# Enigmatisms/NeRF

Measured on AMD Instinct MI355X. Metric: rays/s (64+128 samples), 800x800, higher is better.
Workload: dtype bf16

## Files before the change

nerf_amd/csrc/mlp_core.h:

```cpp
#pragma once
#include "device_common.h"
#include "host_common.h"
#include "mlp_layout.h"

extern __shared__ __attribute__((aligned(16))) char smem[];

namespace {


struct PBF16 {
    using BReg = bf16x8;
    static constexpr int PREC = NERF_AMD_BF16;
    static constexpr int NW = MLP_NW_BF16;
    static constexpr int NT = 1;
    static constexpr int FRAG_BYTES = 1024;
    static constexpr int FPC = MLP_CHUNK_BYTES / FRAG_BYTES;
    using AReg = bf16x8;
    static constexpr int DEPTH = 4;
    static DEVINL AReg load_a(uint32_t frag_addr) { return *reinterpret_cast<const bf16x8*>(smem + frag_addr); }
    static DEVINL f32x16 mma(const AReg& a, const BReg& b, f32x16 acc) {
        return __builtin_amdgcn_mfma_f32_32x32x16_bf16(a, b, acc, 0, 0, 0);
    }
    template <int POS>
    static DEVINL f32x16 mma_pos(const AReg& a, const BReg& b, f32x16 acc) {
// ... 111 lines not shown
    const uint32_t m = __builtin_bit_cast(uint32_t, __builtin_elementwise_max(m01, m23));
    const uint32_t top = (m & 0xffffu) > (m >> 16) ? (m & 0xffffu) : (m >> 16);
    const uint32_t ex = top >> 7;
    return ex > 8u ? ex - 7u : 1u;
}
DEVINL u32x2 f8_encode_group(const bf16x8& v, uint32_t E) {
    const float scale = __builtin_bit_cast(float, E << 23);
    const u32x4 d = __builtin_bit_cast(u32x4, v);
    s16x2 lo = {0, 0}, hi = {0, 0};
    lo = __builtin_amdgcn_cvt_scalef32_pk_fp8_bf16(lo, __builtin_bit_cast(bf16x2, (uint32_t)d[0]), scale, false);
    lo = __builtin_amdgcn_cvt_scalef32_pk_fp8_bf16(lo, __builtin_bit_cast(bf16x2, (uint32_t)d[1]), scale, true);
    hi = __builtin_amdgcn_cvt_scalef32_pk_fp8_bf16(hi, __builtin_bit_cast(bf16x2, (uint32_t)d[2]), scale, false);
    hi = __builtin_amdgcn_cvt_scalef32_pk_fp8_bf16(hi, __builtin_bit_cast(bf16x2, (uint32_t)d[3]), scale, true);
    u32x2 r = {__builtin_bit_cast(uint32_t, lo), __builtin_bit_cast(uint32_t, hi)};
    return r;
}
DEVINL bf16x8 f8_decode_group(uint32_t lo, uint32_t hi, uint32_t E) {
    const float scale = __builtin_bit_cast(float, E << 23);
    const bf16x2 p0 = __builtin_amdgcn_cvt_scalef32_pk_bf16_fp8(lo, scale, false), p1 = __builtin_amdgcn_cvt_scalef32_pk_bf16_fp8(lo, scale, true);
    const bf16x2 p2 = __builtin_amdgcn_cvt_scalef32_pk_bf16_fp8(hi, scale, false), p3 = __builtin_amdgcn_cvt_scalef32_pk_bf16_fp8(hi, scale, true);
    bf16x8 r = {p0[0], p0[1], p1[0], p1[1], p2[0], p2[1], p3[0], p3[1]};
    return r;
}
DEVINL void f8_store_group(char* sub_base, int kg, int lane, const u32x2& v, uint32_t E, uint32_t scale_rec) {
    u32x2* dst = reinterpret_cast<u32x2*>(sub_base + (kg >> 1) * 1024 + lane * 16 + (kg & 1) * 8);
    __builtin_nontemporal_store(v, dst);
    *reinterpret_cast<unsigned char*>(smem + scale_rec + lane * 16 + kg) = (unsigned char)E;
}
DEVINL void f8_flush_scales(char* sub_base, int lane, uint32_t scale_rec) {
    const f32x4 v = *reinterpret_cast<const f32x4*>(smem + scale_rec + lane * 16);
    *reinterpret_cast<f32x4*>(sub_base + F8_SCALE_OFF + lane * 16) = v;
}

template <class P, int NSLOT = MLP_NSLOT>
struct WeightStream {
    static constexpr int LPW = (MLP_CHUNK_BYTES / 1024) / P::NW;
    const char* src;
    uint32_t n_chunks;
    uint32_t load_idx;
    uint32_t load_slot;
    uint32_t cur;
    uint32_t cur_slot;
    uint32_t wave_lds;
    typename P::AReg q[P::DEPTH];
    static DEVINL void dummy_sink(const bf16x8& d) { asm volatile("" ::"v"(d)); }
    template <class T> static DEVINL void dummy_sink(const T& d) { asm volatile("" ::"v"(d.lo), "v"(d.hi)); }
    DEVINL void issue() {
        const char* g = src + (size_t)load_idx * MLP_CHUNK_BYTES;
        const uint32_t dst = __builtin_amdgcn_readfirstlane(load_slot * MLP_CHUNK_BYTES + wave_lds);
#pragma unroll
        for (int i = 0; i < LPW; ++i) {
            unsigned keep;
            asm volatile("s_mov_b32 %0, m0\n\ts_mov_b32 m0, %2\n\ts_nop 0\n\tglobal_load_lds_dwordx4 %1, off\n\ts_mov_b32 m0, %0"
                         : "=&s"(keep)
                         : "v"(g + i * 1024), "s"(dst + i * 1024)
                         : "memory");
        }
        load_idx = (load_idx + 1 == n_chunks) ? 0u : load_idx + 1;
        load_slot = (load_slot + 1 == NSLOT) ? 0u : load_slot + 1;
    }
    static constexpr bool TWO_GROUPS = P::NW > 4;
    static constexpr int INFLIGHT = (TWO_GROUPS ? NSLOT - 5 : NSLOT - 4) * LPW;
    uint32_t late;

    DEVINL void init(const void* packed, uint32_t nchunks) {
        static_assert(NSLOT >= 6, "the protocol needs at least 6 ring slots");
        const int lane = lane_id();
        const int wave = __builtin_amdgcn_readfirstlane((int)(threadIdx.x >> 6));
        src = reinterpret_cast<const char*>(packed) + (size_t)wave * LPW * 1024 + lane * 16;
        wave_lds = wave * LPW * 1024;
        n_chunks = nchunks;
        load_idx = 0; load_slot = 0;
        cur_slot = 0;
        cur = lane * 16;
        late = __builtin_amdgcn_readfirstlane((P::NW > 4 && wave >= P::NW / 2) ? 1 : 0);
#pragma unroll
        for (int i = 0; i < NSLOT - 2; ++i) issue();
        asm volatile("s_waitcnt vmcnt(%0)" ::"n"(INFLIGHT) : "memory");
        __builtin_amdgcn_s_barrier();
        asm volatile("" ::: "memory");
#pragma unroll
        for (int i = 0; i < P::DEPTH; ++i) q[i] = P::load_a(cur + i * P::FRAG_BYTES);
        if (!late) {
            __builtin_amdgcn_s_barrier();
            asm volatile("" ::: "memory");
            issue();
        }
    }
    template <int F>
    DEVINL typename P::AReg next() {
        const typename P::AReg a = q[F % P::DEPTH];
        constexpr int G = F + P::DEPTH;
        if (G % P::FPC == 0) {
            cur_slot = (cur_slot + 1 == NSLOT) ? 0u : cur_slot + 1;
            cur = cur_slot * MLP_CHUNK_BYTES + lane_id() * 16;
            boundary<(G / P::FPC) & 1>();
        }
        q[F % P::DEPTH] = P::load_a(cur + (G % P::FPC) * P::FRAG_BYTES);
        return a;
    }
    template <int PARITY>
    DEVINL void boundary() {
        if constexpr (!TWO_GROUPS && PARITY != 0) {
            issue();
            return;
        }
        asm volatile("s_waitcnt vmcnt(%0)" ::"n"(INFLIGHT) : "memory");
        asm volatile("s_cmp_lg_u32 %0, %1\n\ts_cbranch_scc1 .Lnobar%=\n\ts_barrier\n.Lnobar%=:" ::"s"(__builtin_amdgcn_readfirstlane(late)), "n"(PARITY) : "memory", "scc");
        issue();
    }
    DEVINL void drain() {
        if (late) __builtin_amdgcn_s_barrier();
        asm volatile("s_waitcnt vmcnt(0)" ::: "memory");
    }
};

template <class P, int F0, int N, class WS, int I = 0>
DEVINL void skip_frags(WS& ws) {
    if constexpr (I < N) {
        const typename P::AReg a = ws.template next<F0 + I>();
        WS::dummy_sink(a);
        skip_frags<P, F0, N, WS, I + 1>(ws);
    }
}

// ... 135 lines not shown
```

nerf_amd/csrc/mlp_kernels.hip:

```cpp
#include "mlp_core.h"

namespace {

template <class P, int L, int NKG>
DEVINL void encode(float x, float y, float z, int h, typename P::BReg (&B)[NKG]) {
    if constexpr (P::FAST_PE) {
        float sv[3], cv[3];
        sincos_quadrant(x, sv[0], cv[0]); sincos_quadrant(y, sv[1], cv[1]); sincos_quadrant(z, sv[2], cv[2]);
#pragma unroll
        for (int f = 0; f < L; ++f) {
#pragma unroll
            for (int c = 0; c < 3; ++c) {
                const int q = 3 * f + c;
                P::set(B[q >> 3], q & 7, h ? cv[c] : sv[c]);
                if (f + 1 < L) {
                    const float s2 = 2.0f * sv[c];
                    const float ns = s2 * cv[c];
                    const float nc = __builtin_fmaf(-s2, sv[c], 1.0f);
                    sv[c] = ns; cv[c] = nc;
                }
            }
        }
#pragma unroll
        for (int q = 3 * L; q < 8 * NKG; ++q) {
// ... 143 lines not shown
    }
    float zv;
    if (s.z) zv = s.z[n * s.z_stride + si];
    else {
        const float uu = s.u ? s.u[n * s.S + si] : philox_u_strat(s.rng_seed, n + s.rng_ray_offset, si);
        zv = s.z_base[si] + uu * s.z_jitter;
    }
    r.x = ox + zv * r.dx; r.y = oy + zv * r.dy; r.z = oz + zv * r.dz;
    if (s.contract) contract_position(r);
    return r;
}

struct IpeSample { float mu[3], var[3], dx, dy, dz; };
DEVINL IpeSample fetch_sample_ipe(const nerf_amd_samples& s, int64_t m) {
    IpeSample r;
    int64_t n; int si;
    split_sample_index(s, m, n, si);
    const float* ry = s.rays + n * 6;
    const float* zz = s.z + n * s.z_stride + si;
    const float rr = s.ipe_radius;
    const ConeMoments c = cone_moments(zz[0], zz[1], (float)((double)rr * (double)rr));
    const float dn = s.ipe_dir_norm[0];
#pragma unroll
    for (int k = 0; k < 3; ++k) cone_mean_cov(c, ry[k], ry[3 + k], dn, r.mu[k], r.var[k]);
    r.dx = ry[3]; r.dy = ry[4]; r.dz = ry[5];
    if (s.contract) {
        Sample p{r.mu[0], r.mu[1], r.mu[2], 0.0f, 0.0f, 0.0f};
        contract_position(p);
        r.mu[0] = p.x; r.mu[1] = p.y; r.mu[2] = p.z;
    }
    return r;
}

constexpr uint32_t LDS_BIAS = MLP_RING_BYTES;
constexpr uint32_t LDS_STASH = MLP_RING_BYTES + 9216;
template <class P> constexpr uint32_t lds_dir() { return LDS_STASH + P::NW * P::NT * 4 * P::BREG_LDS; }
template <class P> constexpr uint32_t lds_tile() { return lds_dir<P>() + P::NW * P::NT * 1024; }
template <class P> constexpr uint32_t lds_total() { return lds_tile<P>() + P::NW * P::NT * 32 * 32 + P::NW * P::NT * 8 + 64; }

DEVINL void load_biases(const void* packed, size_t stream_bytes, int n_bias, uint32_t lds_off = MLP_RING_BYTES) {
    const float* b = reinterpret_cast<const float*>(reinterpret_cast<const char*>(packed) + stream_bytes);
    float* dst = reinterpret_cast<float*>(smem + lds_off);
    for (int i = threadIdx.x; i < n_bias; i += blockDim.x) dst[i] = b[i];
    __syncthreads();
}

struct ActDump {
    char* base;
    unsigned long long layer_stride;
    char* mask_base;
    unsigned long long mask_layer_stride;
};
template <class P>
DEVINL void dump_breg(const ActDump& d, int layer, int64_t subtile, int kg, int lane, const typename P::BReg& r) {
#ifndef ABL_NODUMPST
    P::store_global(d.base + (size_t)layer * d.layer_stride + ((size_t)subtile * 16 + kg) * (size_t)P::BREG_LDS, lane, r);
#endif
}

template <class P> constexpr uint32_t lds_maskacc() { return lds_total<P>(); }
template <class P> constexpr uint32_t lds_total_train() { return lds_total<P>() + P::NW * 2 * P::NT * 1024; }
template <class P> constexpr uint32_t lds_scaleacc() { return lds_total_train<P>(); }
template <class P> constexpr uint32_t lds_total_train_f8() { return lds_total_train<P>() + P::NW * 2 * P::NT * 1024; }
template <class P, bool F8>
DEVINL void dump_hidden(const ActDump& d, uint32_t sacc_wave, int layer, int64_t subtile, int t, int kg, int lane, const typename P::BReg& r) {
    if constexpr (F8) {
        const uint32_t E = f8_group_exponent<false>(r);
        f8_store_group(d.base + (size_t)layer * d.layer_stride + (size_t)subtile * F8_SUB_BYTES, kg, lane, f8_encode_group(r, E), E,
                       sacc_wave + ((layer & 1) * P::NT + t) * 1024);
    } else {
        dump_breg<P>(d, layer, subtile, kg, lane, r);
    }
}
DEVINL uint32_t breg_bits(const bf16x8& v) {
    typedef __attribute__((ext_vector_type(4))) uint32_t u32x4;
    const u32x4 d = __builtin_bit_cast(u32x4, v);
    uint32_t m = 0;
#pragma unroll
    for (int i = 0; i < 4; ++i) {
        const uint32_t x = d[i];
        uint32_t on;
        asm("v_pk_min_u16 %0, %1, %2" : "=v"(on) : "v"(x), "v"(0x00010001u));
        m |= on << i;
    }
    return m;
}
DEVINL uint32_t breg_bits(const f32x8& v) {
    uint32_t m = 0;
#pragma unroll
    for (int e = 0; e < 8; ++e) m |= (v[e] > 0.0f ? 1u : 0u) << ((e >> 1) + 16 * (e & 1));
    return m;
}
template <class P>
DEVINL void mask_or(uint32_t acc_wave, int layer, int t, int kg, int lane, const typename P::BReg& v) {
    unsigned* w = reinterpret_cast<unsigned*>(smem + acc_wave + ((layer & 1) * P::NT + t) * 1024 + lane * 16 + (kg >> 2) * 4);
    __hip_atomic_fetch_or(w, breg_bits(v) << (4 * (kg & 3)), __ATOMIC_RELAXED, __HIP_MEMORY_SCOPE_WORKGROUP);
}
template <class P, bool F8 = false>
DEVINL void mask_flush(const ActDump& d, uint32_t acc_wave, int layer, int64_t sub0, int lane, uint32_t sacc_wave = 0) {
    asm volatile("" ::: "memory");
#pragma unroll
    for (int t = 0; t < P::NT; ++t) {
        f32x4* rec = reinterpret_cast<f32x4*>(smem + acc_wave + ((layer & 1) * P::NT + t) * 1024 + lane * 16);
        const f32x4 v = *rec;
        *reinterpret_cast<f32x4*>(d.mask_base + (size_t)layer * d.mask_layer_stride + (size_t)(sub0 + t) * 1024 + lane * 16) = v;
        *rec = f32x4{0.0f, 0.0f, 0.0f, 0.0f};
        if constexpr (F8)
            f8_flush_scales(d.base + (size_t)layer * d.layer_stride + (size_t)(sub0 + t) * F8_SUB_BYTES, lane, sacc_wave + ((layer & 1) * P::NT + t) * 1024);
    }
    asm volatile("" ::: "memory");
}
template <class P>
DEVINL void mask_acc_init(uint32_t acc_wave, int lane) {
#pragma unroll
    for (int i = 0; i < 2 * P::NT; ++i) *reinterpret_cast<f32x4*>(smem + acc_wave + i * 1024 + lane * 16) = f32x4{0.0f, 0.0f, 0.0f, 0.0f};
}

template <class P, bool TRAIN, bool F8 = false>
__global__ __launch_bounds__(P::NW * 64) void proposal_kernel(const void* __restrict__ packed, nerf_amd_samples s,
                                                              float* __restrict__ density, ActDump dump) {
    using L = PropLayout;
    using BReg = typename P::BReg;
    constexpr int FPC = P::FPC;
    load_biases(packed, L::stream_bytes(P::PREC), L::N_BIAS);
    WeightStream<P, MLP_NSLOT> ws;
    ws.init(packed, L::N_FRAGS / FPC);
    const int lane = lane_id(), h = lane >> 5, j = lane & 31;
    const int wave = __builtin_amdgcn_readfirstlane((int)(threadIdx.x >> 6));
    constexpr int NT = P::NT;
    constexpr int TS = P::NW * NT * 32;
    const int64_t n_tiles = (s.M + TS - 1) / TS;
    const uint32_t bias0 = MLP_RING_BYTES;
    const uint32_t macc = lds_maskacc<P>() + wave * 2 * NT * 1024;
    const uint32_t sacc = lds_scaleacc<P>() + wave * 2 * NT * 1024;
    if constexpr (TRAIN) mask_acc_init<P>(macc, lane);

    for (int64_t tile = blockIdx.x; tile < n_tiles; tile += gridDim.x) {
        int64_t m[NT];
        BReg enc[NT][4];
        if constexpr (NT == 2 && P::FAST_PE) {
            m[0] = tile * TS + (wave * NT) * 32 + j;
            m[1] = m[0] + 32;
            const int64_t mo = h ? m[1] : m[0];
            const Sample sm = fetch_sample(s, mo < s.M ? mo : s.M - 1, false);
            encode_pair<P, 10, 4>(sm.x, sm.y, sm.z, enc[0], enc[1]);
            half_swap_groups<4>(enc[0], enc[1]);
            if constexpr (TRAIN) {
#pragma unroll
                for (int t = 0; t < NT; ++t)
#pragma unroll
                    for (int k = 0; k < 4; ++k) dump_breg<P>(dump, 4, tile * (TS / 32) + wave * NT + t, k, lane, enc[t][k]);
            }
        } else {
#pragma unroll
        for (int t = 0; t < NT; ++t) {
            m[t] = tile * TS + (wave * NT + t) * 32 + j;
            const Sample sm = fetch_sample(s, m[t] < s.M ? m[t] : s.M - 1, false);
            encode<P, 10, 4>(sm.x, sm.y, sm.z, h, enc[t]);
            if constexpr (TRAIN) {
#pragma unroll
                for (int k = 0; k < 4; ++k) dump_breg<P>(dump, 4, tile * (TS / 32) + wave * NT + t, k, lane, enc[t][k]);
            }
        }
        }
        BReg a[NT][16], b[NT][16];
        int lay = 0, lay_pend = 0;
        const int64_t sub0 = tile * (TS / 32) + wave * NT;
        auto put = [&](BReg (&buf)[NT][16], int layer, int fb, int t, const f32x16& acc, int half) {
            buf[t][2 * fb + half] = to_breg_half<P, true>(acc, half);
            if constexpr (TRAIN) {
                dump_hidden<P, F8>(dump, sacc, layer, sub0 + t, t, 2 * fb + half, lane, buf[t][2 * fb + half]);
                mask_or<P>(macc, layer, t, 2 * fb + half, lane, buf[t][2 * fb + half]);
            }
        };
        auto OA = [&](int fb, int t, const f32x16& acc, int half) { put(a, lay, fb, t, acc, half); };
        auto OB = [&](int fb, int t, const f32x16& acc, int half) { put(b, lay, fb, t, acc, half); };
        auto OA_pend = [&](int fb, int t, const f32x16& acc, int half) { put(a, lay_pend, fb, t, acc, half); };
        auto OB_pend = [&](int fb, int t, const f32x16& acc, int half) { put(b, lay_pend, fb, t, acc, half); };
        auto IN_A = [&](int kg, int t) -> BReg { return a[t][kg]; };
        Deferred<P, 6, 2> d = dense<P, 4, 8, L::START[0]>(ws, bias0 + L::BIAS_OFF[0] * 4,
            [&](int kg, int t) -> BReg { return enc[t][kg]; }, OA, NoPrev{});
        static_assert(L::START[1] % (2 * FPC) == L::START[3] % (2 * FPC), "chunk parity");
        auto IN_B = [&](int kg, int t) -> BReg { return b[t][kg]; };
#pragma unroll 1
        for (int r = 0; r < 2; ++r) {
            lay_pend = lay; lay = 1 + 2 * r;
            d = dense<P, 16, 8, L::START[1]>(ws, bias0 + (L::BIAS_OFF[1] + r * 512) * 4, IN_A, OB, prev_of(d, OA_pend));
            if constexpr (TRAIN) mask_flush<P, F8>(dump, macc, lay_pend, sub0, lane, sacc);
            if (r == 0) {
                lay_pend = lay; lay = 2;
                d = dense<P, 16, 8, L::START[2]>(ws, bias0 + L::BIAS_OFF[2] * 4, IN_B, OA, prev_of(d, OB_pend));
                if constexpr (TRAIN) mask_flush<P, F8>(dump, macc, lay_pend, sub0, lane, sacc);
            }
        }
        lay_pend = lay;
        float dens[NT];
        auto OH = [&](int, int t, const f32x16& acc, int half) { if (half == 0) dens[t] = acc[0]; };
        dense<P, 16, 1, L::START[4]>(ws, bias0 + L::BIAS_OFF[4] * 4, IN_B, OH, prev_of(d, OB_pend)).flush(OH);
        if constexpr (TRAIN) mask_flush<P, F8>(dump, macc, lay_pend, sub0, lane, sacc);
#pragma unroll
        for (int t = 0; t < NT; ++t)
            if (h == 0 && m[t] < s.M) density[m[t]] = dens[t];
    }
    ws.drain();
}

constexpr uint32_t lds_total_narrow() { return MLP_RING_BYTES + 9216; }
template <class P>
__global__ __launch_bounds__(P::NW * 64) void proposal128_kernel(const void* __restrict__ packed, nerf_amd_samples s, float* __restrict__ density) {
    using L = PropLayout128;
    using BReg = typename P::BReg;
    constexpr int HK = L::HK, HFB = L::HFB;
    load_biases(packed, L::stream_bytes(P::PREC), L::N_BIAS);
    WeightStream<P, MLP_NSLOT> ws;
    ws.init(packed, L::N_FRAGS / P::FPC);
    const int lane = lane_id(), h = lane >> 5, j = lane & 31;
    const int wave = __builtin_amdgcn_readfirstlane((int)(threadIdx.x >> 6));
    constexpr int NT = P::NT;
    constexpr int TS = P::NW * NT * 32;
    const int64_t n_tiles = (s.M + TS - 1) / TS;
    const uint32_t bias0 = MLP_RING_BYTES;
    for (int64_t tile = blockIdx.x; tile < n_tiles; tile += gridDim.x) {
        int64_t m[NT];
        BReg a[NT][HK], b[NT][HK];
        auto OA = [&](int fb, int t, const f32x16& acc, int half) { a[t][2 * fb + half] = to_breg_half<P, true>(acc, half); };
        auto OB = [&](int fb, int t, const f32x16& acc, int half) { b[t][2 * fb + half] = to_breg_half<P, true>(acc, half); };
// ... 19 lines not shown
            d = dense<P, 4, HFB, L::START[0]>(ws, bias0 + L::BIAS_OFF[0] * 4, [&](int kg, int t) -> BReg { return enc[t][kg]; }, OA, NoPrev{});
        }
        d = dense<P, HK, HFB, L::START[1]>(ws, bias0 + L::BIAS_OFF[1] * 4, IN_A, OB, prev_of(d, OA));
        d = dense<P, HK, HFB, L::START[2]>(ws, bias0 + L::BIAS_OFF[2] * 4, IN_B, OA, prev_of(d, OB));
        d = dense<P, HK, HFB, L::START[3]>(ws, bias0 + L::BIAS_OFF[3] * 4, IN_A, OB, prev_of(d, OA));
        float dens[NT];
        auto OH = [&](int, int t, const f32x16& acc, int half) { if (half == 0) dens[t] = acc[0]; };
        dense<P, HK, 1, L::START[4]>(ws, bias0 + L::BIAS_OFF[4] * 4, IN_B, OH, prev_of(d, OB)).flush(OH);
        skip_frags<P, L::USED_FRAGS, L::N_FRAGS - L::USED_FRAGS>(ws);
#pragma unroll
        for (int t = 0; t < NT; ++t)
            if (h == 0 && m[t] < s.M) density[m[t]] = dens[t];
    }
    ws.drain();
}

struct FusedComposite {
    float* rgb;
    float* depth;
    float* weights;
    int white_bkg;
    float near, far;
};

template <class P, bool TRAIN, bool IPE = false, bool F8 = false, bool FUSED = false>
__global__ __launch_bounds__(P::NW * 64) void mip_kernel(const void* __restrict__ packed, nerf_amd_samples s,
                                                         float* __restrict__ rgbo, FusedComposite fc, ActDump dump) {
    using L = MipLayout;
    using BReg = typename P::BReg;
    constexpr int FPC = P::FPC;
#ifdef MLP_CLOCKPROBE
    const uint64_t probe_c0 = __builtin_readcyclecounter(), probe_r0 = __builtin_amdgcn_s_memrealtime();
#endif
    if constexpr (FUSED) { if (threadIdx.x < 16) reinterpret_cast<unsigned*>(smem + lds_tile<P>() + P::NW * P::NT * 32 * 32 + P::NW * P::NT * 8)[threadIdx.x] = 0u; }
    load_biases(packed, L::stream_bytes(P::PREC), L::N_BIAS);
    WeightStream<P, MLP_NSLOT> ws;
    ws.init(packed, L::N_FRAGS / FPC);
    const int lane = lane_id(), h = lane >> 5, j = lane & 31;
    const int wave = __builtin_amdgcn_readfirstlane((int)(threadIdx.x >> 6));
    constexpr int NT = P::NT;
    constexpr int TS = P::NW * NT * 32;
    const int64_t n_tiles = (s.M + TS - 1) / TS;
    const uint32_t bias0 = LDS_BIAS;
    const uint32_t macc = lds_maskacc<P>() + wave * 2 * NT * 1024;
    const uint32_t sacc = lds_scaleacc<P>() + wave * 2 * NT * 1024;
    if constexpr (TRAIN) mask_acc_init<P>(macc, lane);
    const uint32_t enc_lds0 = LDS_STASH + wave * NT * 4 * P::BREG_LDS + lane * 16;
    const uint32_t dir_lds0 = lds_dir<P>() + wave * NT * 1024 + lane * 16;
    auto enc_lds = [&](int t) -> uint32_t { return enc_lds0 + t * 4 * P::BREG_LDS; };
    auto dir_lds = [&](int t) -> uint32_t { return dir_lds0 + t * 1024; };

    for (int64_t tile = blockIdx.x; tile < n_tiles; tile += gridDim.x) {
        int64_t m[NT];
        BReg a[NT][16], b[NT][16];
        int lay = 0, lay_pend = 0;
        const int64_t sub0 = tile * (TS / 32) + wave * NT;
        auto put = [&](BReg (&buf)[NT][16], int layer, int fb, int t, const f32x16& acc, int half) {
            buf[t][2 * fb + half] = to_breg_half<P, true>(acc, half);
            if constexpr (TRAIN) {
                dump_hidden<P, F8>(dump, sacc, layer, sub0 + t, t, 2 * fb + half, lane, buf[t][2 * fb + half]);
                mask_or<P>(macc, layer, t, 2 * fb + half, lane, buf[t][2 * fb + half]);
            }
        };
        auto OA = [&](int fb, int t, const f32x16& acc, int half) { put(a, lay, fb, t, acc, half); };
        auto OB = [&](int fb, int t, const f32x16& acc, int half) { put(b, lay, fb, t, acc, half); };
        auto OA_pend = [&](int fb, int t, const f32x16& acc, int half) { put(a, lay_pend, fb, t, acc, half); };
        auto OB_pend = [&](int fb, int t, const f32x16& acc, int half) { put(b, lay_pend, fb, t, acc, half); };
        auto IN_A = [&](int kg, int t) -> BReg { return a[t][kg]; };
        Deferred<P, 6, 2> d;
        {
            BReg enc[NT][4];
            if constexpr (NT == 2 && P::FAST_PE && !IPE && !FUSED) {
                m[0] = tile * TS + (wave * NT) * 32 + j;
                m[1] = m[0] + 32;
                const int64_t mo = h ? m[1] : m[0];
                const Sample sm = fetch_sample(s, mo < s.M ? mo : s.M - 1, true);
                encode_pair<P, 10, 4>(sm.x, sm.y, sm.z, enc[0], enc[1]);
                half_swap_groups<4>(enc[0], enc[1]);
                uint32_t d0[3] = {__builtin_bit_cast(uint32_t, sm.dx), __builtin_bit_cast(uint32_t, sm.dy), __builtin_bit_cast(uint32_t, sm.dz)};
                uint32_t d1[3] = {d0[0], d0[1], d0[2]};
#pragma unroll
// ... 80 lines not shown
                dump_breg<P>(dump, 8, sub0 + t, 5, lane, denc[t][1]);
            }
        }
        BReg c[NT][8];
        auto OC = [&](int fb, int t, const f32x16& acc, int half) {
            c[t][2 * fb + half] = to_breg_half<P, true>(acc, half);
            if constexpr (TRAIN) {
                dump_hidden<P, F8>(dump, sacc, 7, sub0 + t, t, 2 * fb + half, lane, c[t][2 * fb + half]);
                mask_or<P>(macc, 7, t, 2 * fb + half, lane, c[t][2 * fb + half]);
            }
        };
        const auto dc = dense<P, 18, 4, L::START[8]>(ws, bias0 + L::BIAS_OFF[8] * 4,
            [&](int kg, int t) -> BReg { if (kg < 16) return a[t][kg < 16 ? kg : 0]; return denc[t][kg >= 16 ? kg - 16 : 0]; },
            OC, prev_of(dsig, OSIG));
        float r[NT], g[NT], bl[NT];
        auto ORGB = [&](int, int t, const f32x16& acc, int half) { if (half == 0) { r[t] = acc[0]; g[t] = acc[1]; bl[t] = acc[2]; } };
        dense<P, 8, 1, L::START[9]>(ws, bias0 + L::BIAS_OFF[9] * 4,
            [&](int kg, int t) -> BReg { return c[t][kg]; }, ORGB, prev_of(dc, OC)).flush(ORGB);
        if constexpr (TRAIN) mask_flush<P, F8>(dump, macc, 7, sub0, lane, sacc);
        f32x4 o[NT];
#pragma unroll
        for (int t = 0; t < NT; ++t) {
            o[t][0] = 1.0f / (1.0f + expf(-r[t]));
            o[t][1] = 1.0f / (1.0f + expf(-g[t]));
            o[t][2] = 1.0f / (1.0f + expf(-bl[t]));
            o[t][3] = sigma[t];
            if constexpr (!FUSED) {
                if (h == 0 && m[t] < s.M) *reinterpret_cast<f32x4*>(rgbo + m[t] * 4) = o[t];
            }
        }
        if constexpr (FUSED) {
            const int S = s.S;
            const int spr = S >> 5;
            char* tb = smem + lds_tile<P>();
            f32x4* t_ca = reinterpret_cast<f32x4*>(tb);
            u32x4* t_pz = reinterpret_cast<u32x4*>(tb + TS * 16);
            double* t_seg = reinterpret_cast<double*>(tb + TS * 32);
            unsigned* tickets = reinterpret_cast<unsigned*>(tb + TS * 32 + (TS / 32) * 8);
            {
                const int tt = (NT > 1) ? h : 0;
                const bool live = (NT > 1) || h == 0;
                const float k0 = (*reinterpret_cast<const f32x4*>(smem + dir_lds(0)))[3];
                const float k1 = (NT > 1) ? (*reinterpret_cast<const f32x4*>(smem + dir_lds(NT - 1)))[3] : 0.0f;
                float cr, cg, cb, sg, zn, dl;
                if (NT > 1) {
                    const float s0 = __shfl(o[NT - 1][0], j, 64), s1 = __shfl(o[NT - 1][1], j, 64), s2 = __shfl(o[NT - 1][2], j, 64),
                                s3 = __shfl(o[NT - 1][3], j, 64), sz = __shfl(k1, j, 64), d0 = __shfl(k0, j + 32, 64);
                    cr = h ? s0 : o[0][0]; cg = h ? s1 : o[0][1]; cb = h ? s2 : o[0][2]; sg = h ? s3 : o[0][3];
                    zn = h ? sz : k0;
                    dl = h ? k1 : d0;
                } else {
                    cr = o[0][0]; cg = o[0][1]; cb = o[0][2]; sg = o[0][3]; zn = k0; dl = __shfl(k0, j + 32, 64);
                }
                const float mm = expf(-fmaxf(sg, 0.0f) * dl);
                const float al = live ? 1.0f - mm : 0.0f;
                const double p = live ? (double)(mm + 1e-10f) : 1.0;
                const double incl = seg32_incl_scan_mul(p);
                double excl = wave_shift_up1(incl, 1.0);
                if (lane == 32) excl = 1.0;
                const int sub = wave * NT + tt;
                if (live) {
                    const int ts = sub * 32 + j;
                    t_ca[ts] = f32x4{cr, cg, cb, al};
                    const u32x2 eb = __builtin_bit_cast(u32x2, excl);
                    t_pz[ts] = u32x4{eb[0], eb[1], __builtin_bit_cast(uint32_t, zn), 0u};
                }
                if (j == 31 && live) t_seg[sub] = incl;
// ... 404 lines not shown
        dense<P, 16, 1, L::START[17]>(ws, bias0 + L::BIAS_OFF[17] * 4, IN_B, OSPEC, prev_of(d, OB_pend)).flush(OSPEC);
#pragma unroll
        for (int t = 0; t < NT; ++t) {
            const float d0 = __shfl(keep[t][0], j + 32, 64), d1 = __shfl(keep[t][1], j + 32, 64), d2 = __shfl(keep[t][2], j + 32, 64),
                        dens = __shfl(keep[t][3], j + 32, 64);
            if (h == 0 && m[t] < s.M) {
                auto sig = [](float v) { return 1.0f / (1.0f + expf(-v)); };
                f32x4 o;
                if (flags & NERF_AMD_REF_SRGB) {
                    o[0] = srgb_from_linear(sig(sr[t]) * sig(keep[t][0]) + sig(d0 - SRGB_LOG3));
                    o[1] = srgb_from_linear(sig(sg[t]) * sig(keep[t][1]) + sig(d1 - SRGB_LOG3));
                    o[2] = srgb_from_linear(sig(sb[t]) * sig(keep[t][2]) + sig(d2 - SRGB_LOG3));
                } else {
                    o[0] = sig(sr[t]) * sig(keep[t][0]) + sig(d0);
                    o[1] = sig(sg[t]) * sig(keep[t][1]) + sig(d1);
                    o[2] = sig(sb[t]) * sig(keep[t][2]) + sig(d2);
                }
                o[3] = dens;
                *reinterpret_cast<f32x4*>(rgbo + m[t] * 4) = o;
                if constexpr (TRAIN) { float* ax = aux + m[t] * 16; ax[11] = sr[t]; ax[12] = sg[t]; ax[13] = sb[t]; ax[14] = 0.0f; ax[15] = 0.0f; }
            }
        }
    }
    ws.drain();
}

int grid_for(int64_t n_tiles) {
    const int n_cu = nerf_host::cu_count();
    return (int)(n_tiles < n_cu ? n_tiles : n_cu);
}

int allow_dynamic_lds(const void* fn, size_t lds) { return nerf_host::allow_dynamic_lds(fn, lds); }

template <class P, class Lay, bool TRAIN = false, bool F8 = false, class K, class... Extra>
int launch(K kernel, const void* packed, const nerf_amd_samples& s, float* out, hipStream_t st, Extra... extra) {
    constexpr int TS = P::NW * P::NT * 32;
    const int64_t n_tiles = (s.M + TS - 1) / TS;
    if (n_tiles == 0) return 0;
    const size_t lds = F8 ? lds_total_train_f8<P>() : (TRAIN ? lds_total_train<P>() : lds_total<P>());
    if (int e = allow_dynamic_lds(reinterpret_cast<const void*>(kernel), lds)) return e;
    hipLaunchKernelGGL(kernel, dim3(grid_for(n_tiles)), dim3(P::NW * 64), lds, st, packed, s, out, extra...);
    return (int)hipGetLastError();
}
const ActDump NO_DUMP{nullptr, 0ull, nullptr, 0ull};

using PB16 = PBF16W;

}

#ifndef MLP_TU
#define MLP_TU 0
#endif
#if MLP_TU == 0 || MLP_TU == 1
int mlp_launch_proposal(const void* packed, int precision, const nerf_amd_samples& s, float* density, hipStream_t st) {
    if (precision == NERF_AMD_BF16) return launch<PB16, PropLayout>(proposal_kernel<PB16, false>, packed, s, density, st, NO_DUMP);
    return launch<PF32, PropLayout>(proposal_kernel<PF32, false>, packed, s, density, st, NO_DUMP);
}
#endif
#if MLP_TU == 0 || MLP_TU == 2
int mlp_launch_mip(const void* packed, int precision, const nerf_amd_samples& s, float* rgbo, hipStream_t st) {
    const FusedComposite off{nullptr, nullptr, nullptr, 0, 0.0f, 1.0f};
    if (s.ipe) {
        if (precision == NERF_AMD_BF16) return launch<PB16, MipLayout>(mip_kernel<PB16, false, true>, packed, s, rgbo, st, off, NO_DUMP);
        return launch<PF32, MipLayout>(mip_kernel<PF32, false, true>, packed, s, rgbo, st, off, NO_DUMP);
    }
    if (precision == NERF_AMD_BF16) return launch<PB16, MipLayout>(mip_kernel<PB16, false>, packed, s, rgbo, st, off, NO_DUMP);
    return launch<PF32, MipLayout>(mip_kernel<PF32, false>, packed, s, rgbo, st, off, NO_DUMP);
}
int mlp_launch_mip128(const void* packed, int precision, const nerf_amd_samples& s, float* rgbo, hipStream_t st) {
    if (precision == NERF_AMD_BF16) return launch<PB16, MipLayout128>(mip128_kernel<PB16>, packed, s, rgbo, st);
    return launch<PF32, MipLayout128>(mip128_kernel<PF32>, packed, s, rgbo, st);
}
int mlp_launch_mip_composite(const void* packed, int precision, const nerf_amd_samples& s, float* rgb, float* depth, float* weights,
                             int white_bkg, float near, float far, hipStream_t st) {
    const FusedComposite fc{rgb, depth, weights, white_bkg, near, far};
    if (precision == NERF_AMD_BF16) return launch<PB16, MipLayout>(mip_kernel<PB16, false, false, false, true>, packed, s, (float*)nullptr, st, fc, NO_DUMP);
    return launch<PF32, MipLayout>(mip_kernel<PF32, false, false, false, true>, packed, s, (float*)nullptr, st, fc, NO_DUMP);
}
#endif
#if MLP_TU == 0 || MLP_TU == 1
template <class P>
static int launch_proposal128(const void* packed, const nerf_amd_samples& s, float* density, hipStream_t st) {
    constexpr int TS = P::NW * P::NT * 32;
    const int64_t n_tiles = (s.M + TS - 1) / TS;
    if (n_tiles == 0) return 0;
    const size_t lds = lds_total_narrow();
    if (int e = allow_dynamic_lds(reinterpret_cast<const void*>(proposal128_kernel<P>), lds)) return e;
    hipLaunchKernelGGL(proposal128_kernel<P>, dim3(grid_for(n_tiles)), dim3(P::NW * 64), lds, st, packed, s, density);
    return (int)hipGetLastError();
}
int mlp_launch_proposal128(const void* packed, int precision, const nerf_amd_samples& s, float* density, hipStream_t st) {
    if (precision == NERF_AMD_BF16) return launch_proposal128<PBF16N>(packed, s, density, st);
    return launch_proposal128<PF32>(packed, s, density, st);
}
#endif
#if MLP_TU == 0 || MLP_TU == 1
size_t mlp_train_layer_stride(int precision, int64_t M) {
    const int64_t ts = (precision != NERF_AMD_F32) ? (int64_t)PB16::NW * PB16::NT * 32 : (int64_t)PF32::NW * PF32::NT * 32;
    const int64_t n_sub = ((M + ts - 1) / ts) * (ts / 32);
    return (size_t)n_sub * 16 * (precision != NERF_AMD_F32 ? 1024 : 2048);
}
size_t mlp_train_mask_stride(int precision, int64_t M) { return mlp_train_layer_stride(precision, M) / (16 * (precision != NERF_AMD_F32 ? 1024 : 2048)) * 1024; }
#else
size_t mlp_train_layer_stride(int precision, int64_t M);
size_t mlp_train_mask_stride(int precision, int64_t M);
#endif
static ActDump make_dump(void* dump, int precision, int64_t M, int slots) {
    const unsigned long long ls = mlp_train_layer_stride(precision, M);
    return ActDump{reinterpret_cast<char*>(dump), ls, reinterpret_cast<char*>(dump) + (size_t)slots * ls, (unsigned long long)mlp_train_mask_stride(precision, M)};
}
#if MLP_TU == 0 || MLP_TU == 1
int mlp_launch_proposal_train(const void* packed, int precision, const nerf_amd_samples& s, float* density, void* dump, hipStream_t st) {
    if (precision == NERF_AMD_BF16_F8) {
        const ActDump d8 = make_dump(dump, NERF_AMD_BF16, s.M, PROP_DUMP_SLOTS);
        return launch<PB16, PropLayout, true, true>(proposal_kernel<PB16, true, true>, packed, s, density, st, d8);
    }
    const ActDump d = make_dump(dump, precision, s.M, PROP_DUMP_SLOTS);
    if (precision == NERF_AMD_BF16) return launch<PBF16, PropLayout, true>(proposal_kernel<PBF16, true>, packed, s, density, st, d);
    return launch<PF32, PropLayout, true>(proposal_kernel<PF32, true>, packed, s, density, st, d);
}
#endif
#if MLP_TU == 0 || MLP_TU == 2
int mlp_launch_mip_train(const void* packed, int precision, const nerf_amd_samples& s, float* rgbo, void* dump, hipStream_t st) {
    const FusedComposite off{nullptr, nullptr, nullptr, 0, 0.0f, 1.0f};
    if (precision == NERF_AMD_BF16_F8) {
        const ActDump d8 = make_dump(dump, NERF_AMD_BF16, s.M, MIP_DUMP_SLOTS);
        if (s.ipe) return launch<PB16, MipLayout, true, true>(mip_kernel<PB16, true, true, true>, packed, s, rgbo, st, off, d8);
        return launch<PB16, MipLayout, true, true>(mip_kernel<PB16, true, false, true>, packed, s, rgbo, st, off, d8);
    }
    const ActDump d = make_dump(dump, precision, s.M, MIP_DUMP_SLOTS);
    if (s.ipe) {
        if (precision == NERF_AMD_BF16) return launch<PB16, MipLayout, true>(mip_kernel<PB16, true, true>, packed, s, rgbo, st, off, d);
        return launch<PF32, MipLayout, true>(mip_kernel<PF32, true, true>, packed, s, rgbo, st, off, d);
    }
    if (precision == NERF_AMD_BF16) return launch<PB16, MipLayout, true>(mip_kernel<PB16, true>, packed, s, rgbo, st, off, d);
    return launch<PF32, MipLayout, true>(mip_kernel<PF32, true>, packed, s, rgbo, st, off, d);
}

#endif
#if MLP_TU == 0 || MLP_TU == 3
template <class P, bool TRAIN>
static int launch_ref(const void* packed, const nerf_amd_samples& s, float* rgbo, float* normal, const float* bn_noise, ActDump dump, float* aux,
                      int flags, hipStream_t st, unsigned long long seed = 0, const unsigned long long* seed_dev = nullptr, float noise_std = 0.0f) {
    constexpr int TS = P::NW * P::NT * 32;
    const int64_t n_tiles = (s.M + TS - 1) / TS;
    if (n_tiles == 0) return 0;
    const size_t lds = ref_lds_total<P>();
    if (int e = allow_dynamic_lds(reinterpret_cast<const void*>(ref_kernel<P, TRAIN>), lds)) return e;
    hipLaunchKernelGGL((ref_kernel<P, TRAIN>), dim3(grid_for(n_tiles)), dim3(P::NW * 64), lds, st, packed, s, rgbo, normal, bn_noise, dump, aux, flags, seed, seed_dev, noise_std);
    return (int)hipGetLastError();
}
int mlp_launch_ref(const void* packed, int precision, const nerf_amd_samples& s, float* rgbo, float* normal, const float* bn_noise,
                   int flags, hipStream_t st) {
    if (precision == NERF_AMD_BF16) return launch_ref<PB16, false>(packed, s, rgbo, normal, bn_noise, NO_DUMP, nullptr, flags, st);
    return launch_ref<PF32, false>(packed, s, rgbo, normal, bn_noise, NO_DUMP, nullptr, flags, st);
}
int mlp_launch_ref_train(const void* packed, int precision, const nerf_amd_samples& s, float* rgbo, float* normal, const float* bn_noise,
                         void* dump, float* aux, int flags, hipStream_t st, unsigned long long seed, const unsigned long long* seed_dev, float noise_std) {
    const ActDump d = make_dump(dump, precision, s.M, REF_DUMP_SLOTS);
#ifndef REF_TRAIN_WIDE
    if (precision == NERF_AMD_BF16) return launch_ref<PBF16, true>(packed, s, rgbo, normal, bn_noise, d, aux, flags, st, seed, seed_dev, noise_std);
#endif
    if (precision == NERF_AMD_BF16) return launch_ref<PB16, true>(packed, s, rgbo, normal, bn_noise, d, aux, flags, st, seed, seed_dev, noise_std);
    return launch_ref<PF32, true>(packed, s, rgbo, normal, bn_noise, d, aux, flags, st, seed, seed_dev, noise_std);
}
#endif
```

Measured before the change: 9.433 million.

## Keep tail weight fragments resident in LDS and compute per-kernel LDS plans

Adds an LDS plan that sizes each kernel's shared memory exactly and uses the leftover LDS to hold a resident range of weight fragments. Those fragments are copied once at kernel start, and later fragment loads read them directly instead of streaming them through the ring. This cuts per-tile global-to-LDS weight traffic and ring synchronisation for the resident layers. The render proposal kernel also unrolls its hidden layers into a straight sequence that matches the resident indexing. In exchange, LDS use per workgroup grows, which may lower occupancy, and startup gains a full load and barrier.

Result: no change. 9.505 million, median of 6 (+0.8%).

```diff
diff --git a/nerf_amd/csrc/mlp_core.h b/nerf_amd/csrc/mlp_core.h
--- a/nerf_amd/csrc/mlp_core.h
+++ b/nerf_amd/csrc/mlp_core.h
@@ -167,9 +167,14 @@
     *reinterpret_cast<f32x4*>(sub_base + F8_SCALE_OFF + lane * 16) = v;
 }
 
-template <class P, int NSLOT = MLP_NSLOT>
+template <class P, int NSLOT = MLP_NSLOT, int NFRAGS = 0, int NRES = 0, uint32_t RES_LDS = 0>
 struct WeightStream {
     static constexpr int LPW = (MLP_CHUNK_BYTES / 1024) / P::NW;
+    static constexpr int NSTREAM = NFRAGS - NRES;
+    static constexpr int RES_PIECES = NRES * P::FRAG_BYTES / 1024;
+    static_assert(NRES >= 0 && (NRES == 0 || (NRES % (2 * P::FPC) == 0 && NFRAGS % (2 * P::FPC) == 0 && NSTREAM >= 2 * P::FPC)),
+                  "the resident range and the streamed remainder are even numbers of whole chunks");
+    static_assert(RES_PIECES % P::NW == 0 && RES_LDS % 16 == 0, "every wave copies the same number of resident pieces");
     const char* src;
     uint32_t n_chunks;
     uint32_t load_idx;
@@ -180,17 +185,18 @@
     typename P::AReg q[P::DEPTH];
     static DEVINL void dummy_sink(const bf16x8& d) { asm volatile("" ::"v"(d)); }
     template <class T> static DEVINL void dummy_sink(const T& d) { asm volatile("" ::"v"(d.lo), "v"(d.hi)); }
+    static DEVINL void glds(const char* g, uint32_t dst) {
+        unsigned keep;
+        asm volatile("s_mov_b32 %0, m0\n\ts_mov_b32 m0, %2\n\ts_nop 0\n\tglobal_load_lds_dwordx4 %1, off\n\ts_mov_b32 m0, %0"
+                     : "=&s"(keep)
+                     : "v"(g), "s"(dst)
+                     : "memory");
+    }
     DEVINL void issue() {
         const char* g = src + (size_t)load_idx * MLP_CHUNK_BYTES;
         const uint32_t dst = __builtin_amdgcn_readfirstlane(load_slot * MLP_CHUNK_BYTES + wave_lds);
 #pragma unroll
-        for (int i = 0; i < LPW; ++i) {
-            unsigned keep;
-            asm volatile("s_mov_b32 %0, m0\n\ts_mov_b32 m0, %2\n\ts_nop 0\n\tglobal_load_lds_dwordx4 %1, off\n\ts_mov_b32 m0, %0"
-                         : "=&s"(keep)
-                         : "v"(g + i * 1024), "s"(dst + i * 1024)
-                         : "memory");
-        }
+        for (int i = 0; i < LPW; ++i) glds(g + i * 1024, dst + i * 1024);
         load_idx = (load_idx + 1 == n_chunks) ? 0u : load_idx + 1;
         load_slot = (load_slot + 1 == NSLOT) ? 0u : load_slot + 1;
     }
@@ -198,6 +204,10 @@
     static constexpr int INFLIGHT = (TWO_GROUPS ? NSLOT - 5 : NSLOT - 4) * LPW;
     uint32_t late;
 
+    DEVINL void init(const void* packed) {
+        static_assert(NFRAGS > 0 && NSTREAM % P::FPC == 0, "stream length");
+        init(packed, NSTREAM / P::FPC);
+    }
     DEVINL void init(const void* packed, uint32_t nchunks) {
         static_assert(NSLOT >= 6, "the protocol needs at least 6 ring slots");
         const int lane = lane_id();
@@ -209,6 +219,15 @@
         cur_slot = 0;
         cur = lane * 16;
         late = __builtin_amdgcn_readfirstlane((P::NW > 4 && wave >= P::NW / 2) ? 1 : 0);
+        if constexpr (NRES > 0) {
+            const char* g = reinterpret_cast<const char*>(packed) + (size_t)NSTREAM * P::FRAG_BYTES + (size_t)wave * 1024 + lane * 16;
+#pragma unroll 1
+            for (int i = 0; i < RES_PIECES / P::NW; ++i)
+                glds(g + (size_t)i * P::NW * 1024, __builtin_amdgcn_readfirstlane(RES_LDS + (uint32_t)(i * P::NW + wave) * 1024u));
+            asm volatile("s_waitcnt vmcnt(0)" ::: "memory");
+            __builtin_amdgcn_s_barrier();
+            asm volatile("" ::: "memory");
+        }
 #pragma unroll
         for (int i = 0; i < NSLOT - 2; ++i) issue();
         asm volatile("s_waitcnt vmcnt(%0)" ::"n"(INFLIGHT) : "memory");
@@ -226,6 +245,11 @@
     DEVINL typename P::AReg next() {
         const typename P::AReg a = q[F % P::DEPTH];
         constexpr int G = F + P::DEPTH;
+        static_assert(NRES == 0 || (F >= 0 && F < NFRAGS), "with a resident range F is the absolute fragment index");
+        if constexpr (NRES > 0 && G >= NSTREAM && G < NFRAGS) {
+            q[F % P::DEPTH] = P::load_a(RES_LDS + (uint32_t)(G - NSTREAM) * P::FRAG_BYTES + lane_id() * 16);
+            return a;
+        }
         if (G % P::FPC == 0) {
             cur_slot = (cur_slot + 1 == NSLOT) ? 0u : cur_slot + 1;
             cur = cur_slot * MLP_CHUNK_BYTES + lane_id() * 16;
diff --git a/nerf_amd/csrc/mlp_kernels.hip b/nerf_amd/csrc/mlp_kernels.hip
--- a/nerf_amd/csrc/mlp_kernels.hip
+++ b/nerf_amd/csrc/mlp_kernels.hip
@@ -199,6 +199,34 @@
     return r;
 }
 
+#ifndef MLP_NSLOT_RENDER
+#define MLP_NSLOT_RENDER MLP_NSLOT
+#endif
+constexpr uint32_t LDS_CU_BYTES = 160 * 1024;
+template <class P, class L, int NSLOT_, bool MIP, bool TRAIN, bool F8, bool FUSED, int MAX_RES>
+struct LdsPlan {
+    static constexpr int NSLOT = NSLOT_;
+    static constexpr uint32_t BIAS = MLP_CHUNK_BYTES * NSLOT;
+    static constexpr uint32_t STASH = BIAS + ((L::N_BIAS * 4 + 15) & ~15u);
+    static constexpr uint32_t DIR = STASH + (MIP ? P::NW * P::NT * 4 * P::BREG_LDS : 0);
+    static constexpr uint32_t TILE = DIR + (MIP ? P::NW * P::NT * 1024 : 0);
+    static constexpr uint32_t TICKETS = TILE + P::NW * P::NT * 32 * 32 + P::NW * P::NT * 8;
+    static constexpr uint32_t MASK = FUSED ? TICKETS + 64 : TILE;
+    static constexpr uint32_t SCALE = MASK + (TRAIN ? P::NW * 2 * P::NT * 1024 : 0);
+    static constexpr uint32_t RES = SCALE + (F8 ? P::NW * 2 * P::NT * 1024 : 0);
+    static_assert(RES <= LDS_CU_BYTES && RES % 16 == 0, "LDS plan");
+    static constexpr int FIT = (int)((LDS_CU_BYTES - RES) / (2 * MLP_CHUNK_BYTES)) * 2 * P::FPC;
+    static constexpr int CAP = MAX_RES > 0 ? MAX_RES / (2 * P::FPC) * (2 * P::FPC) : 0;
+    static constexpr int NRES = FIT < CAP ? FIT : CAP;
+    static constexpr uint32_t TOTAL = RES + NRES * P::FRAG_BYTES;
+    using Stream = WeightStream<P, NSLOT, L::N_FRAGS, NRES, RES>;
+};
+template <class P, bool TRAIN, bool F8>
+using PropPlan = LdsPlan<P, PropLayout, TRAIN ? MLP_NSLOT : MLP_NSLOT_RENDER, false, TRAIN, F8, false,
+                         TRAIN ? PropLayout::N_FRAGS - PropLayout::START[4] - P::DEPTH : PropLayout::N_FRAGS - 2 * P::FPC>;
+template <class P, bool TRAIN, bool F8, bool FUSED>
+using MipPlan = LdsPlan<P, MipLayout, TRAIN ? MLP_NSLOT : MLP_NSLOT_RENDER, true, TRAIN, F8, FUSED, MipLayout::N_FRAGS - MipLayout::START[7] - P::DEPTH>;
+
 constexpr uint32_t LDS_BIAS = MLP_RING_BYTES;
 constexpr uint32_t LDS_STASH = MLP_RING_BYTES + 9216;
 template <class P> constexpr uint32_t lds_dir() { return LDS_STASH + P::NW * P::NT * 4 * P::BREG_LDS; }
@@ -225,10 +253,6 @@
 #endif
 }
 
-template <class P> constexpr uint32_t lds_maskacc() { return lds_total<P>(); }
-template <class P> constexpr uint32_t lds_total_train() { return lds_total<P>() + P::NW * 2 * P::NT * 1024; }
-template <class P> constexpr uint32_t lds_scaleacc() { return lds_total_train<P>(); }
-template <class P> constexpr uint32_t lds_total_train_f8() { return lds_total_train<P>() + P::NW * 2 * P::NT * 1024; }
 template <class P, bool F8>
 DEVINL void dump_hidden(const ActDump& d, uint32_t sacc_wave, int layer, int64_t subtile, int t, int kg, int lane, const typename P::BReg& r) {
     if constexpr (F8) {
@@ -287,20 +311,23 @@
 __global__ __launch_bounds__(P::NW * 64) void proposal_kernel(const void* __restrict__ packed, nerf_amd_samples s,
                                                               float* __restrict__ density, ActDump dump) {
     using L = PropLayout;
+    using Plan = PropPlan<P, TRAIN, F8>;
     using BReg = typename P::BReg;
     constexpr int FPC = P::FPC;
-    load_biases(packed, L::stream_bytes(P::PREC), L::N_BIAS);
-    WeightStream<P, MLP_NSLOT> ws;
-    ws.init(packed, L::N_FRAGS / FPC);
+    load_biases(packed, L::stream_bytes(P::PREC), L::N_BIAS, Plan::BIAS);
+    typename Plan::Stream ws;
+    ws.init(packed);
     const int lane = lane_id(), h = lane >> 5, j = lane & 31;
     const int wave = __builtin_amdgcn_readfirstlane((int)(threadIdx.x >> 6));
     constexpr int NT = P::NT;
     constexpr int TS = P::NW * NT * 32;
     const int64_t n_tiles = (s.M + TS - 1) / TS;
-    const uint32_t bias0 = MLP_RING_BYTES;
-    const uint32_t macc = lds_maskacc<P>() + wave * 2 * NT * 1024;
-    const uint32_t sacc = lds_scaleacc<P>() + wave * 2 * NT * 1024;
+    const uint32_t bias0 = Plan::BIAS;
+    const uint32_t macc = Plan::MASK + wave * 2 * NT * 1024;
+    const uint32_t sacc = Plan::SCALE + wave * 2 * NT * 1024;
     if constexpr (TRAIN) mask_acc_init<P>(macc, lane);
+    int once = 1;
+    asm volatile("" : "+s"(once));
 
     for (int64_t tile = blockIdx.x; tile < n_tiles; tile += gridDim.x) {
         int64_t m[NT];
@@ -347,8 +374,9 @@
         auto IN_A = [&](int kg, int t) -> BReg { return a[t][kg]; };
         Deferred<P, 6, 2> d = dense<P, 4, 8, L::START[0]>(ws, bias0 + L::BIAS_OFF[0] * 4,
             [&](int kg, int t) -> BReg { return enc[t][kg]; }, OA, NoPrev{});
+        auto IN_B = [&](int kg, int t) -> BReg { return b[t][kg]; };
+        if constexpr (TRAIN) {
         static_assert(L::START[1] % (2 * FPC) == L::START[3] % (2 * FPC), "chunk parity");
-        auto IN_B = [&](int kg, int t) -> BReg { return b[t][kg]; };
 #pragma unroll 1
         for (int r = 0; r < 2; ++r) {
             lay_pend = lay; lay = 1 + 2 * r;
@@ -359,6 +387,14 @@
                 d = dense<P, 16, 8, L::START[2]>(ws, bias0 + L::BIAS_OFF[2] * 4, IN_B, OA, prev_of(d, OB_pend));
                 if constexpr (TRAIN) mask_flush<P, F8>(dump, macc, lay_pend, sub0, lane, sacc);
             }
+        }
+        } else {
+#pragma unroll 1
+            for (int r = 0; r < once; ++r) {
+                d = dense<P, 16, 8, L::START[1]>(ws, bias0 + L::BIAS_OFF[1] * 4, IN_A, OB, prev_of(d, OA_pend));
+                d = dense<P, 16, 8, L::START[2]>(ws, bias0 + L::BIAS_OFF[2] * 4, IN_B, OA, prev_of(d, OB_pend));
+            }
+            d = dense<P, 16, 8, L::START[3]>(ws, bias0 + L::BIAS_OFF[3] * 4, IN_A, OB, prev_of(d, OA_pend));
         }
         lay_pend = lay;
         float dens[NT];
@@ -444,21 +480,22 @@
 #ifdef MLP_CLOCKPROBE
     const uint64_t probe_c0 = __builtin_readcyclecounter(), probe_r0 = __builtin_amdgcn_s_memrealtime();
 #endif
-    if constexpr (FUSED) { if (threadIdx.x < 16) reinterpret_cast<unsigned*>(smem + lds_tile<P>() + P::NW * P::NT * 32 * 32 + P::NW * P::NT * 8)[threadIdx.x] = 0u; }
-    load_biases(packed, L::stream_bytes(P::PREC), L::N_BIAS);
-    WeightStream<P, MLP_NSLOT> ws;
-    ws.init(packed, L::N_FRAGS / FPC);
+    using Plan = MipPlan<P, TRAIN, F8, FUSED>;
+    if constexpr (FUSED) { if (threadIdx.x < 16) reinterpret_cast<unsigned*>(smem + Plan::TICKETS)[threadIdx.x] = 0u; }
+    load_biases(packed, L::stream_bytes(P::PREC), L::N_BIAS, Plan::BIAS);
+    typename Plan::Stream ws;
+    ws.init(packed);
     const int lane = lane_id(), h = lane >> 5, j = lane & 31;
     const int wave = __builtin_amdgcn_readfirstlane((int)(threadIdx.x >> 6));
     constexpr int NT = P::NT;
     constexpr int TS = P::NW * NT * 32;
     const int64_t n_tiles = (s.M + TS - 1) / TS;
-    const uint32_t bias0 = LDS_BIAS;
-    const uint32_t macc = lds_maskacc<P>() + wave * 2 * NT * 1024;
-    const uint32_t sacc = lds_scaleacc<P>() + wave * 2 * NT * 1024;
+    const uint32_t bias0 = Plan::BIAS;
+    const uint32_t macc = Plan::MASK + wave * 2 * NT * 1024;
+    const uint32_t sacc = Plan::SCALE + wave * 2 * NT * 1024;
     if constexpr (TRAIN) mask_acc_init<P>(macc, lane);
-    const uint32_t enc_lds0 = LDS_STASH + wave * NT * 4 * P::BREG_LDS + lane * 16;
-    const uint32_t dir_lds0 = lds_dir<P>() + wave * NT * 1024 + lane * 16;
+    const uint32_t enc_lds0 = Plan::STASH + wave * NT * 4 * P::BREG_LDS + lane * 16;
+    const uint32_t dir_lds0 = Plan::DIR + wave * NT * 1024 + lane * 16;
     auto enc_lds = [&](int t) -> uint32_t { return enc_lds0 + t * 4 * P::BREG_LDS; };
     auto dir_lds = [&](int t) -> uint32_t { return dir_lds0 + t * 1024; };
 
@@ -605,7 +642,7 @@
         if constexpr (FUSED) {
             const int S = s.S;
             const int spr = S >> 5;
-            char* tb = smem + lds_tile<P>();
+            char* tb = smem + Plan::TILE;
             f32x4* t_ca = reinterpret_cast<f32x4*>(tb);
             u32x4* t_pz = reinterpret_cast<u32x4*>(tb + TS * 16);
             double* t_seg = reinterpret_cast<double*>(tb + TS * 32);
@@ -1076,12 +1113,13 @@
 
 int allow_dynamic_lds(const void* fn, size_t lds) { return nerf_host::allow_dynamic_lds(fn, lds); }
 
-template <class P, class Lay, bool TRAIN = false, bool F8 = false, class K, class... Extra>
+template <class P, uint32_t LDS, class K, class... Extra>
 int launch(K kernel, const void* packed, const nerf_amd_samples& s, float* out, hipStream_t st, Extra... extra) {
     constexpr int TS = P::NW * P::NT * 32;
     const int64_t n_tiles = (s.M + TS - 1) / TS;
     if (n_tiles == 0) return 0;
-    const size_t lds = F8 ? lds_total_train_f8<P>() : (TRAIN ? lds_total_train<P>() : lds_total<P>());
+    static_assert(LDS <= LDS_CU_BYTES, "LDS per workgroup");
+    const size_t lds = LDS;
     if (int e = allow_dynamic_lds(reinterpret_cast<const void*>(kernel), lds)) return e;
     hipLaunchKernelGGL(kernel, dim3(grid_for(n_tiles)), dim3(P::NW * 64), lds, st, packed, s, out, extra...);
     return (int)hipGetLastError();
@@ -1097,29 +1135,29 @@
 #endif
 #if MLP_TU == 0 || MLP_TU == 1
 int mlp_launch_proposal(const void* packed, int precision, const nerf_amd_samples& s, float* density, hipStream_t st) {
-    if (precision == NERF_AMD_BF16) return launch<PB16, PropLayout>(proposal_kernel<PB16, false>, packed, s, density, st, NO_DUMP);
-    return launch<PF32, PropLayout>(proposal_kernel<PF32, false>, packed, s, density, st, NO_DUMP);
+    if (precision == NERF_AMD_BF16) return launch<PB16, PropPlan<PB16, false, false>::TOTAL>(proposal_kernel<PB16, false>, packed, s, density, st, NO_DUMP);
+    return launch<PF32, PropPlan<PF32, false, false>::TOTAL>(proposal_kernel<PF32, false>, packed, s, density, st, NO_DUMP);
 }
 #endif
 #if MLP_TU == 0 || MLP_TU == 2
 int mlp_launch_mip(const void* packed, int precision, const nerf_amd_samples& s, float* rgbo, hipStream_t st) {
     const FusedComposite off{nullptr, nullptr, nullptr, 0, 0.0f, 1.0f};
     if (s.ipe) {
-        if (precision == NERF_AMD_BF16) return launch<PB16, MipLayout>(mip_kernel<PB16, false, true>, packed, s, rgbo, st, off, NO_DUMP);
-        return launch<PF32, MipLayout>(mip_kernel<PF32, false, true>, packed, s, rgbo, st, off, NO_DUMP);
-    }
-    if (precision == NERF_AMD_BF16) return launch<PB16, MipLayout>(mip_kernel<PB16, false>, packed, s, rgbo, st, off, NO_DUMP);
-    return launch<PF32, MipLayout>(mip_kernel<PF32, false>, packed, s, rgbo, st, off, NO_DUMP);
+        if (precision == NERF_AMD_BF16) return launch<PB16, MipPlan<PB16, false, false, false>::TOTAL>(mip_kernel<PB16, false, true>, packed, s, rgbo, st, off, NO_DUMP);
+        return launch<PF32, MipPlan<PF32, false, false, false>::TOTAL>(mip_kernel<PF32, false, true>, packed, s, rgbo, st, off, NO_DUMP);
+    }
+    if (precision == NERF_AMD_BF16) return launch<PB16, MipPlan<PB16, false, false, false>::TOTAL>(mip_kernel<PB16, false>, packed, s, rgbo, st, off, NO_DUMP);
+    return launch<PF32, MipPlan<PF32, false, false, false>::TOTAL>(mip_kernel<PF32, false>, packed, s, rgbo, st, off, NO_DUMP);
 }
 int mlp_launch_mip128(const void* packed, int precision, const nerf_amd_samples& s, float* rgbo, hipStream_t st) {
-    if (precision == NERF_AMD_BF16) return launch<PB16, MipLayout128>(mip128_kernel<PB16>, packed, s, rgbo, st);
-    return launch<PF32, MipLayout128>(mip128_kernel<PF32>, packed, s, rgbo, st);
+    if (precision == NERF_AMD_BF16) return launch<PB16, lds_total<PB16>()>(mip128_kernel<PB16>, packed, s, rgbo, st);
+    return launch<PF32, lds_total<PF32>()>(mip128_kernel<PF32>, packed, s, rgbo, st);
 }
 int mlp_launch_mip_composite(const void* packed, int precision, const nerf_amd_samples& s, float* rgb, float* depth, float* weights,
                              int white_bkg, float near, float far, hipStream_t st) {
     const FusedComposite fc{rgb, depth, weights, white_bkg, near, far};
-    if (precision == NERF_AMD_BF16) return launch<PB16, MipLayout>(mip_kernel<PB16, false, false, false, true>, packed, s, (float*)nullptr, st, fc, NO_DUMP);
-    return launch<PF32, MipLayout>(mip_kernel<PF32, false, false, false, true>, packed, s, (float*)nullptr, st, fc, NO_DUMP);
+    if (precision == NERF_AMD_BF16) return launch<PB16, MipPlan<PB16, false, false, true>::TOTAL>(mip_kernel<PB16, false, false, false, true>, packed, s, (float*)nullptr, st, fc, NO_DUMP);
+    return launch<PF32, MipPlan<PF32, false, false, true>::TOTAL>(mip_kernel<PF32, false, false, false, true>, packed, s, (float*)nullptr, st, fc, NO_DUMP);
 }
 #endif
 #if MLP_TU == 0 || MLP_TU == 1
@@ -1157,11 +1195,11 @@
 int mlp_launch_proposal_train(const void* packed, int precision, const nerf_amd_samples& s, float* density, void* dump, hipStream_t st) {
     if (precision == NERF_AMD_BF16_F8) {
         const ActDump d8 = make_dump(dump, NERF_AMD_BF16, s.M, PROP_DUMP_SLOTS);
-        return launch<PB16, PropLayout, true, true>(proposal_kernel<PB16, true, true>, packed, s, density, st, d8);
+        return launch<PB16, PropPlan<PB16, true, true>::TOTAL>(proposal_kernel<PB16, true, true>, packed, s, density, st, d8);
     }
     const ActDump d = make_dump(dump, precision, s.M, PROP_DUMP_SLOTS);
-    if (precision == NERF_AMD_BF16) return launch<PBF16, PropLayout, true>(proposal_kernel<PBF16, true>, packed, s, density, st, d);
-    return launch<PF32, PropLayout, true>(proposal_kernel<PF32, true>, packed, s, density, st, d);
+    if (precision == NERF_AMD_BF16) return launch<PBF16, PropPlan<PBF16, true, false>::TOTAL>(proposal_kernel<PBF16, true>, packed, s, density, st, d);
+    return launch<PF32, PropPlan<PF32, true, false>::TOTAL>(proposal_kernel<PF32, true>, packed, s, density, st, d);
 }
 #endif
 #if MLP_TU == 0 || MLP_TU == 2
@@ -1169,16 +1207,16 @@
     const FusedComposite off{nullptr, nullptr, nullptr, 0, 0.0f, 1.0f};
     if (precision == NERF_AMD_BF16_F8) {
         const ActDump d8 = make_dump(dump, NERF_AMD_BF16, s.M, MIP_DUMP_SLOTS);
-        if (s.ipe) return launch<PB16, MipLayout, true, true>(mip_kernel<PB16, true, true, true>, packed, s, rgbo, st, off, d8);
-        return launch<PB16, MipLayout, true, true>(mip_kernel<PB16, true, false, true>, packed, s, rgbo, st, off, d8);
+        if (s.ipe) return launch<PB16, MipPlan<PB16, true, true, false>::TOTAL>(mip_kernel<PB16, true, true, true>, packed, s, rgbo, st, off, d8);
+        return launch<PB16, MipPlan<PB16, true, true, false>::TOTAL>(mip_kernel<PB16, true, false, true>, packed, s, rgbo, st, off, d8);
     }
     const ActDump d = make_dump(dump, precision, s.M, MIP_DUMP_SLOTS);
     if (s.ipe) {
-        if (precision == NERF_AMD_BF16) return launch<PB16, MipLayout, true>(mip_kernel<PB16, true, true>, packed, s, rgbo, st, off, d);
-        return launch<PF32, MipLayout, true>(mip_kernel<PF32, true, true>, packed, s, rgbo, st, off, d);
-    }
-    if (precision == NERF_AMD_BF16) return launch<PB16, MipLayout, true>(mip_kernel<PB16, true>, packed, s, rgbo, st, off, d);
-    return launch<PF32, MipLayout, true>(mip_kernel<PF32, true>, packed, s, rgbo, st, off, d);
+        if (precision == NERF_AMD_BF16) return launch<PB16, MipPlan<PB16, true, false, false>::TOTAL>(mip_kernel<PB16, true, true>, packed, s, rgbo, st, off, d);
+        return launch<PF32, MipPlan<PF32, true, false, false>::TOTAL>(mip_kernel<PF32, true, true>, packed, s, rgbo, st, off, d);
+    }
+    if (precision == NERF_AMD_BF16) return launch<PB16, MipPlan<PB16, true, false, false>::TOTAL>(mip_kernel<PB16, true>, packed, s, rgbo, st, off, d);
+    return launch<PF32, MipPlan<PF32, true, false, false>::TOTAL>(mip_kernel<PF32, true>, packed, s, rgbo, st, off, d);
 }
 
 #endif
```
